# sag111/ContiniousEnvironment_Follower_Leader

Measured on AMD Instinct MI355X. Metric: env-steps/sec at 65,536 parallel envs; 1/2/4/8 MI355X scaling, higher is better.
Workload: dtype f64

## Files before the change

continiousenvironment_follower_leader_amd/_lib.py:

```python
import ctypes as C
import os
import subprocess

from . import abi

_PKG = os.path.dirname(os.path.abspath(__file__))
_ROOT = os.path.dirname(_PKG)
SO_PATH = os.path.join(_PKG, "libftl_hip.so")
SOURCES = [os.path.join(_PKG, "csrc", "ftl_abi.hip"), os.path.join(_PKG, "csrc", "ftl_device.hpp"),
           os.path.join(_PKG, "csrc", "ftl_frames_group.hpp"), os.path.join(_PKG, "csrc", "ftl_aux.hpp"), os.path.join(_PKG, "csrc", "ftl_gazebo.hpp"), os.path.join(_ROOT, "include", "ftl_gazebo.h"), os.path.join(_PKG, "csrc", "ftl_scenario.cpp"),
           os.path.join(_PKG, "csrc", "ftl_scenario_dev.hpp"),
           os.path.join(_PKG, "csrc", "ftl_scenario_core.hpp"),
           os.path.join(_PKG, "csrc", "ftl_crmath.hpp"),
           os.path.join(_PKG, "csrc", "ftl_render.hpp"),
           os.path.join(_PKG, "csrc", "ftl_snapshot.hpp"),
           os.path.join(_PKG, "csrc", "ftl_restart.hpp"),
           os.path.join(_PKG, "csrc", "ftl_queue.hpp"),
           os.path.join(_PKG, "csrc", "ftl_sampler.hpp"),
           os.path.join(_ROOT, "include", "ftl.h")]
UNITS = [os.path.join(_PKG, "csrc", "ftl_abi.hip"), os.path.join(_PKG, "csrc", "ftl_scenario.cpp")]
HIPCC = os.environ.get("HIPCC", "/opt/rocm/bin/hipcc")
HIPCC_FLAGS = ["--offload-arch=gfx950", "-O3", "-ffp-contract=off", "-fPIC", "-shared", "-std=c++17"]

_LIB = None


def build(force=False, verbose=False):
    stale = (not os.path.exists(SO_PATH)) or any(os.path.getmtime(s) > os.path.getmtime(SO_PATH) for s in SOURCES)
    if force or stale:
        cmd = [HIPCC] + HIPCC_FLAGS + ["-pthread", "-o", SO_PATH] + UNITS
        if verbose:
            print(" ".join(cmd))
        subprocess.check_call(cmd, cwd=os.path.join(_PKG, "csrc"))
    return SO_PATH


class FtlError(RuntimeError):
    pass


def load():
    global _LIB
# ... 106 lines not shown
```

continiousenvironment_follower_leader_amd/csrc/ftl_abi.hip:

```cpp
#include <hip/hip_runtime.h>

#include <cstdio>
#include <cstring>
#include <new>
#include <string>
#include <vector>

#include <cstdlib>
#include <cmath>

#include "ftl_device.hpp"
#include "ftl_frames_group.hpp"
#include "ftl_aux.hpp"

namespace {

thread_local std::string g_err;

int fail(int code, const std::string& msg) { g_err = msg; return code; }

struct Field { const char* name; size_t offset, per_env; int dtype; size_t stride; };

#define FTL_FIELDS(X) \
    X(rb_pos, 1, 4, true) X(rb_dbl, 2, 8, true) X(rb_int, 0, 4, true) X(env_int, 0, 4, true) X(env_dbl, 2, 8, true) \
    X(traj, 1, 4, false) X(hist, 2, 8, false) X(corr, 2, 8, false) X(snap_rects, 0, 4, true) X(snap_win, 0, 4, true) \
    X(traj_bb, 1, 4, false) X(ep_stats, 2, 8, false) X(hist1, 1, 4, false) X(fol_cs, 2, 8, true) X(corr32, 1, 4, false)
#define X(n, dtype, esz, rec) F_##n,
enum { FTL_FIELDS(X) FTL_N_FIELDS };
#undef X
struct FieldSpec { const char* name; int dtype; size_t esz; bool rec; size_t ptr; };
#define X(n, dtype, esz, rec) {#n, dtype, esz, rec, offsetof(FtlDevParams, n)},
constexpr FieldSpec kFields[FTL_N_FIELDS] = {FTL_FIELDS(X)};
#undef X
constexpr int kRecOrder[] = {F_env_int, F_fol_cs, F_rb_pos, F_rb_dbl, F_snap_win, F_snap_rects, F_env_dbl, F_rb_int};

struct Switches {
    int split, no_regroup, g8, one_pass, defer;
    int regroup_every, corr_lds_cap, lds_pad, lds_pad_rays;
    bool print_lds;
};

Switches read_switches() {
    auto tri = [](const char* name, int other) { const char* v = getenv(name); return !v ? -1 : v[0] == '1' ? 1 : v[0] == '0' ? 0 : other; };
    auto num = [](const char* name, int hi) { const char* v = getenv(name); const int p = v ? atoi(v) : 0; return p < 0 ? 0 : (p > hi ? hi : p); };
    return Switches{tri("FTL_SPLIT", 0), tri("FTL_NO_REGROUP", 0), tri("FTL_DEBUG_G8", 0), tri("FTL_RAYS_ONE_PASS", 1), tri("FTL_DEFER", 1),
                    num("FTL_REGROUP_EVERY", INT32_MAX), num("FTL_DEBUG_CORR_LDS_CAP", INT32_MAX), num("FTL_DEBUG_LDS_PAD", 48 * 1024),
                    num("FTL_DEBUG_LDS_PAD_RAYS", 48 * 1024), getenv("FTL_DEBUG_PRINT_LDS") != nullptr};
}

struct Schedule {
    int G, epw, rg_slots;
    int32_t fr_rec_off, fr_rec_stride, fr_pend_off, fr_env_off, fr_defer, fr_lds;
    bool regroup, fits;
};

struct FrameInst { int G; bool reg, xr; };
struct RaysInst { int hm; bool expl, split, capped, one_pass; };
typedef void (*FtlKernel)(const FtlDevParams*, const FtlCall);

}

template <typename T> struct FtlAttached { T v; bool attached; int32_t calls; };
struct FtlRestartScratch { int32_t* scen_idx; int32_t* list; uint8_t* ended; uint8_t* restarted; };

struct ftl_handle {
    FtlDevParams P;
    FtlDevParams* dP;
    bool dirty;
    int device;
    size_t state_bytes;
    Field fields[FTL_N_FIELDS];
    void* mt_mem;
    bool timing;
    std::vector<hipEvent_t> tev;
    size_t tev_used;
    bool bound, have_scen;
    Switches sw;
    Schedule sched;
    int co_envs, cus;
    bool one_pass;
    FtlKernel k_frames[2], k_rays[2]; RaysInst rays[2];
    bool has_aux, has_trk1;
    void* rg_mem;
    int* rg_tot;
    unsigned rg_parity, rg_launches, rg_every;
    hipStream_t side; hipEvent_t ev_fork, ev_join; bool split;
    int win_base, win_count, win_stride;
    float* last_lasers;
    FtlAttached<ftl_episode_queue> queue;
    FtlAttached<ftl_scenario_sampler> sampler;
// ... 51 lines not shown
        REQ(l.history > 0 && l.history <= FTL_HMAX, "laser %d: max_prev_obs must be in 1..%d", k, FTL_HMAX);
        REQ(l.react_obstacles >= 0 && l.react_obstacles <= 3, "laser %d: bad react_to_obstacles", k);
        REQ(l.length > 0, "laser %d: bad laser_length", k);
    }
#undef REQ
    return FTL_OK;
}

int frames_max(const ftl_config& c) { return c.rand_fps_hi > 0 ? c.rand_fps_hi - 1 : c.frames_per_step; }

Schedule plan_schedule(const ftl_config& cfg, int R, int n_envs, int co_envs, int cus, const Switches& sw) {
    Schedule s;
    s.G = (R > 4 || (sw.g8 >= 0 ? sw.g8 == 1 : co_envs <= cus * 4 * 8)) ? 8 : 4;
    s.epw = FTL_WAVE / s.G;
    const int f_max = frames_max(cfg);
    s.fr_defer = (cfg.rand_fps_hi == 0 && f_max >= 2 && f_max <= 16 && cfg.traj_cap <= 65535 && sw.defer != 0) ? 1 : 0;
    size_t o = align_up((size_t)s.epw * cfg.n_static * 16 + (size_t)s.epw * 4 + 32, 16);
    s.fr_rec_stride = (int)align_up((size_t)f_max, 16);
    s.fr_rec_off = (int)o; o += (size_t)s.fr_rec_stride * s.epw;
    s.fr_pend_off = (int)o; o += (size_t)s.epw * (s.fr_defer ? f_max - 1 : 1) * 16;
    s.fr_env_off = (int)o; o += (size_t)s.epw * 4 + 16 + (size_t)s.epw * 16;
    s.fr_lds = (int)o;
    s.fits = o <= 64 * 1024;
    s.rg_slots = cus * 4 * FTL_FRAMESG_WPE;
    s.regroup = (sw.no_regroup >= 0 ? sw.no_regroup == 0 : ((co_envs + s.epw - 1) / s.epw > s.rg_slots || cfg.rand_fps_hi > 0))
                && (n_envs + FTL_RG_BLOCK - 1) / FTL_RG_BLOCK <= 512;
    return s;
}

FrameInst frame_inst(const ftl_config& c, int G, bool xr) { return FrameInst{G, c.n_speed_regime >= 0 || c.n_acc_regime >= 0 || c.rand_fps_hi > 0, xr}; }

bool call_xr(const FtlCall& c) { return (c.flags & (FTL_STEP_NEXT_RESET | FTL_CALL_DEFER_RESET | FTL_CALL_FINISH)) != 0 || c.ended || c.restarted; }

RaysInst rays_inst(int hmax, bool expl, bool capped, bool two_streams, bool one_pass) {
    const int wide = hmax <= 5 ? 5 : FTL_HMAX;
    if (two_streams) return (!expl && hmax > 5 && hmax <= 10) ? RaysInst{10, false, true, capped, false} : RaysInst{wide, true, true, capped, false};
    if (expl) return RaysInst{wide, true, false, capped, false};
    return RaysInst{hmax <= 5 ? 5 : hmax <= 8 ? 8 : hmax <= 10 ? 10 : FTL_HMAX, false, false, capped, one_pass};
}

template <bool XR> FtlKernel frame_kernel_x(int G, bool reg) {
    if (G == 4) return reg ? ftl_frames_group_kernel<4, true, XR> : ftl_frames_group_kernel<4, false, XR>;
    return reg ? ftl_frames_group_kernel<8, true, XR> : ftl_frames_group_kernel<8, false, XR>;
}
FtlKernel frame_kernel(const FrameInst& f) { return f.xr ? frame_kernel_x<true>(f.G, f.reg) : frame_kernel_x<false>(f.G, f.reg); }

template <int HM, bool EXPL, bool SPLIT, bool ONE> FtlKernel rays_kernel_c(bool capped) {
    return capped ? ftl_rays_kernel<HM, EXPL, SPLIT, true, ONE> : ftl_rays_kernel<HM, EXPL, SPLIT, false, ONE>;
}
template <int HM> FtlKernel rays_kernel_1(const RaysInst& r) { return r.one_pass ? rays_kernel_c<HM, false, false, true>(r.capped) : rays_kernel_c<HM, false, false, false>(r.capped); }
FtlKernel rays_kernel(const RaysInst& r) {
    if (r.split) return r.hm == 10 ? rays_kernel_c<10, false, true, false>(r.capped) : r.hm == 5 ? rays_kernel_c<5, true, true, false>(r.capped) : rays_kernel_c<FTL_HMAX, true, true, false>(r.capped);
    if (r.expl) return r.hm == 5 ? rays_kernel_c<5, true, false, false>(r.capped) : rays_kernel_c<FTL_HMAX, true, false, false>(r.capped);
    return r.hm == 5 ? rays_kernel_1<5>(r) : r.hm == 8 ? rays_kernel_1<8>(r) : r.hm == 10 ? rays_kernel_1<10>(r) : rays_kernel_1<FTL_HMAX>(r);
}

int apply_plan(ftl_handle* h, int co_envs) {
    FtlDevParams& P = h->P;
    const ftl_config& c = P.cfg;
    const Schedule s = plan_schedule(c, P.R, P.n_envs, co_envs, h->cus, h->sw);
    if (!s.fits) return fail(FTL_E_INVALID, "the frame kernel needs more than 64 KiB of LDS per wavefront (static rects x frames per step)");
    h->sched = s; h->co_envs = co_envs; h->dirty = true;
    P.fr_rec_off = s.fr_rec_off; P.fr_rec_stride = s.fr_rec_stride; P.fr_pend_off = s.fr_pend_off; P.fr_env_off = s.fr_env_off;
    P.fr_defer = s.fr_defer; P.fr_lds = s.fr_lds;
    bool expl = false, compas = false;
    for (int k = 0; k < c.n_lasers; k++) { compas = compas || c.lasers[k].compas != 0; expl = expl || c.lasers[k].explicit_angles != 0 || c.lasers[k].pad_sectors != 0; }
    for (int i = 0; i < 2; i++) {
        h->k_frames[i] = frame_kernel(frame_inst(c, s.G, i == 1));
        h->rays[i] = rays_inst(P.hmax, expl || compas, P.corr_lds_cap < c.corr_cap, i == 1, h->one_pass);
        h->k_rays[i] = c.n_lasers > 0 ? rays_kernel(h->rays[i]) : nullptr;
    }
    h->has_aux = c.n_aux > 0 || compas; h->has_trk1 = c.has_tracker == 1;
    return FTL_OK;
}

void report_plan(const ftl_handle* h) {
    if (!h->sw.print_lds) return;
    const FtlDevParams& P = h->P;
    fprintf(stderr, "ftl: frame kernel LDS %d B per wavefront, %d lanes per env, %d frames at most, searches %s\n", P.fr_lds, h->sched.G, frames_max(P.cfg), P.fr_defer ? "deferred" : "in frame");
    fprintf(stderr, "ftl: ray kernel LDS %d B per env\n", P.lds_rays);
    char r[2][40] = {"no rays", "no rays"};
    for (int i = 0; i < 2; i++)
        if (h->k_rays[i]) snprintf(r[i], sizeof r[i], "rays<%d,%d,%d,%d,%d>", h->rays[i].hm, h->rays[i].expl, h->rays[i].split, h->rays[i].capped, h->rays[i].one_pass);
    fprintf(stderr, "ftl: kernels frames<%d,%d>, %s on one stream, %s on two; regroup %s every %u, two streams %s\n", h->sched.G, frame_inst(P.cfg, h->sched.G, false).reg,
            r[0], r[1], h->sched.regroup ? "on" : "off", h->rg_every, h->split ? "on" : "off");
}

}

extern "C" {

const char* ftl_last_error(void) { return g_err.c_str(); }

size_t ftl_sizeof_config(void) { return sizeof(ftl_config); }
size_t ftl_sizeof_scenarios(void) { return sizeof(ftl_scenarios); }
size_t ftl_sizeof_outputs(void) { return sizeof(ftl_outputs); }
size_t ftl_sizeof_scen_params(void) { return sizeof(ftl_scen_params); }
size_t ftl_sizeof_final_outputs(void) { return sizeof(ftl_final_outputs); }

int ftl_create(const ftl_config* cfg, int32_t n_envs, int32_t device, ftl_handle** out) {
    if (!cfg || !out) return fail(FTL_E_INVALID, "null argument");
    if (n_envs <= 0) return fail(FTL_E_INVALID, "n_envs must be positive");
    if (device < 0) return fail(FTL_E_INVALID, "device < 0: this library has no CPU path");
    std::string why;
    if (int rc = validate(*cfg, why)) return fail(rc, why);
    ftl_handle* h = new (std::nothrow) ftl_handle();
    if (!h) return fail(FTL_E_DEVICE, "out of host memory");
    h->P.cfg = *cfg;
    for (int k = 0; k < FTL_MAX_LASERS; k++) h->P.cfg.lasers[k].after_tracker = cfg->lasers[k].after_tracker ? 1 : 0;
    h->device = device; h->dirty = true;
    h->sw = read_switches();
    h->split = n_envs >= 8192 && (h->sw.split >= 0 ? h->sw.split == 1 : cfg->rand_fps_hi > 0) && cfg->has_tracker != 1;
    h->rg_every = h->sw.regroup_every > 0 ? (unsigned)h->sw.regroup_every : 4u;
    h->cus = 256;
    (void)hipDeviceGetAttribute(&h->cus, hipDeviceAttributeMultiprocessorCount, device);
    FtlDevParams& P = h->P;
    P.n_envs = n_envs;
    P.R = 2 + cfg->n_bears;
// ... 23 lines not shown
        }
        P.miss_const = miss_ok ? 1 : 0;
        int rb[2] = {0, 0};
        for (int k = 0; k < cfg->n_lasers; k++) {
            const ftl_laser_cfg& l = cfg->lasers[k];
            FtlRaySensor& rs = P.ray_sens[k];
            const int which = l.after_tracker ? 1 : 0, ro = l.react_obstacles;
            rs.count = l.count; rs.rbase = rb[which];
            rs.reach2 = ((float)l.length + 2.0f) * ((float)l.length + 2.0f);
            rs.inv_step = (float)l.count * 0.15915494309189535f; rs.inv_count = 1.0f / (float)l.count;
            rs.off_u = (float)(l.angle_offset * deg2rad) * rs.inv_step;
            rs.slack = 0.022f + 0.01f * (float)l.count * 0.15915494f;
            rs.flags = ((ro == 1 || ro == 2) ? 1u : 0u) | ((ro == 1 || ro == 3) ? 2u : 0u) | (l.react_corridor ? 4u : 0u) | (l.react_green ? 8u : 0u)
                     | (l.explicit_angles ? 16u : 0u) | (which ? 32u : 0u) | (l.compas ? 64u : 0u);
            if (!l.compas) rb[which] += l.count;
        }
        P.inv_nrect_dyn = (65536u + (unsigned)(P.R - 1) - 1u) / (unsigned)(P.R - 1);
        int g = 0;
        for (int which = 0; which < 2; which++) {
            P.pass_base[which] = g; P.pass_lmax[which] = 0.0f;
            for (int k = 0; k < cfg->n_lasers; k++) {
                const ftl_laser_cfg& l = cfg->lasers[k];
                if ((l.after_tracker ? 1 : 0) != which || l.compas) continue;
                P.pass_lmax[which] = fmaxf(P.pass_lmax[which], (float)l.length);
                for (int i = 0; i < l.count && g < FTL_MAX_RAYS; i++, g++) {
                    const double a = l.explicit_angles ? l.ray_angles[i & 7] : l.angle_offset + i * (360.0 / (double)l.count);
                    P.ray_dir[g].c = cos(a * deg2rad); P.ray_dir[g].s = sin(a * deg2rad); P.ray_dir[g].len = l.length;
                }
            }
            P.pass_rays[which] = g - P.pass_base[which];
        }
        P.pass_single = P.pass_rays[0] > 0 && P.pass_rays[1] > 0 ? -1 : (P.pass_rays[1] > 0 ? 1 : 0);
        h->one_pass = P.pass_single >= 0 && h->sw.one_pass != 0;
    }
    if (rays > 1023) { delete h; return fail(FTL_E_INVALID, "more than 1023 rays per env (the candidate list of the ray kernel packs a ray index into 10 bits)"); }
    if (hmax * (P.R - 1) > FTL_WAVE) { delete h; return fail(FTL_E_INVALID, "max_prev_obs x (1 + bears) exceeds one wavefront of snapshot rects"); }
    {
        int w = 0, hcommon = 0;
        for (int k = 0; k < cfg->n_lasers; k++) {
            P.pol_off[k] = -1;
            if (!cfg->lasers[k].in_policy_obs) continue;
            P.pol_off[k] = w; w += width_of(cfg->lasers[k]);
            if (hcommon == 0) hcommon = cfg->lasers[k].history;
            else if (cfg->lasers[k].history != hcommon) hcommon = -1;
        }
        P.pol_width = w; P.pol_h = hcommon;
    }
    const size_t n = (size_t)n_envs;
    size_t per_env[FTL_N_FIELDS];
    per_env[F_rb_pos] = (size_t)P.R * 2; per_env[F_rb_dbl] = (size_t)P.R * FTL_RD_COUNT; per_env[F_rb_int] = (size_t)P.R * FTL_RI_COUNT;
    per_env[F_env_int] = FTL_EI_COUNT; per_env[F_env_dbl] = FTL_ED_COUNT; per_env[F_fol_cs] = 2;
    per_env[F_snap_rects] = (size_t)hmax * (P.R - 1) * 4; per_env[F_snap_win] = (size_t)hmax * 4;
    per_env[F_traj] = (size_t)cfg->traj_cap * 2; per_env[F_traj_bb] = (size_t)(cfg->traj_cap / FTL_TRAJ_BLOCK) * 4;
    per_env[F_hist] = (size_t)cfg->corr_cap * 2; per_env[F_corr] = (size_t)cfg->corr_cap * 4; per_env[F_corr32] = (size_t)cfg->corr_cap * 4;
    per_env[F_hist1] = (size_t)(cfg->has_tracker == 1 ? cfg->hist1_cap : 0) * 2; per_env[F_ep_stats] = FTL_N_METRICS;
    size_t ro = 0;
    for (int i : kRecOrder) {
        ro = align_up(ro, 16);
        h->fields[i] = Field{kFields[i].name, ro, per_env[i], kFields[i].dtype, 0};
        ro += per_env[i] * kFields[i].esz;
    }
    const size_t rec_stride = align_up(ro, 128);
    P.rec_stride = (int32_t)rec_stride;
    for (int i : kRecOrder) h->fields[i].stride = rec_stride;
    size_t cur = rec_stride * n;
    for (int i = 0; i < FTL_N_FIELDS; i++) {
        if (kFields[i].rec) continue;
        cur = align_up(cur, 256);
        h->fields[i] = Field{kFields[i].name, cur, per_env[i], kFields[i].dtype, per_env[i] * kFields[i].esz};
        cur += per_env[i] * kFields[i].esz * n;
    }
    h->state_bytes = align_up(cur, 256);
    {
        const size_t rects = (size_t)cfg->n_static + hmax + (size_t)hmax * (P.R - 2 > 0 ? P.R - 2 : 0) + 1;
        P.corr_lds_cap = cfg->corr_cap < 128 ? cfg->corr_cap : 128;
        if (const int v = h->sw.corr_lds_cap; v >= 2 && v <= cfg->corr_cap && (v & (v - 1)) == 0) P.corr_lds_cap = v;
        const int hm_lds = rays_inst(hmax, true, false, false, false).hm;
        P.lds_rays = (int)((size_t)P.corr_lds_cap * 16 + rects * 20 + (size_t)2 * P.corr_lds_cap * 4 + (size_t)2 * hmax * 20 + 64
                           + (size_t)rays * 16 + (size_t)rays * hm_lds * 4 + (size_t)rays * 4
                           + rects * 8 + 32
                           + (size_t)FTL_PAIR_CAP * 2 + 16);
    }
    P.lds_rays += h->sw.lds_pad_rays;
    if (cfg->traj_cap > 65535 || frames_max(*cfg) > 4095) { delete h; return fail(FTL_E_INVALID, "traj_cap above 65535 or more than 4095 frames per step"); }
    if (apply_plan(h, n_envs)) { delete h; return FTL_E_INVALID; }
    report_plan(h);
    if (P.lds_rays > 64 * 1024) { delete h; return fail(FTL_E_INVALID, "config needs more than 64 KiB of LDS per env"); }
    if (ftl_aux_lds_bytes(*cfg) > 64 * 1024) { delete h; return fail(FTL_E_INVALID, "the compas / lidar / radar sensors of this config need more than 64 KiB of LDS per env"); }
    *out = h;
    return FTL_OK;
}

void ftl_destroy(ftl_handle* h) {
    if (!h) return;
    if (h->dP || h->rg_mem || h->side || h->mt_mem || h->rs.scen_idx) (void)hipSetDevice(h->device);
    if (h->rs.scen_idx) (void)hipFree(h->rs.scen_idx);
    if (h->dP) (void)hipFree(h->dP);
    if (h->mt_mem) (void)hipFree(h->mt_mem);
    for (hipEvent_t ev : h->tev) (void)hipEventDestroy(ev);
    if (h->rg_mem) (void)hipFree(h->rg_mem);
    if (h->side) { (void)hipStreamSynchronize(h->side); (void)hipStreamDestroy(h->side); }
    if (h->ev_fork) (void)hipEventDestroy(h->ev_fork);
    if (h->ev_join) (void)hipEventDestroy(h->ev_join);
    delete h;
}

int32_t ftl_lasers_len(const ftl_handle* h) { return h ? h->P.lasers_len : 0; }

int ftl_get_config(const ftl_handle* h, ftl_config* out) {
    if (!h || !out) return fail(FTL_E_INVALID, "null argument");
// ... 315 lines not shown
```

continiousenvironment_follower_leader_amd/csrc/ftl_device.hpp:

```cpp
#pragma once
#include <hip/hip_runtime.h>
#include <stddef.h>
#include <stdint.h>

#include "../../include/ftl.h"

#define FTL_WAVE 64
#define FTL_HMAX 12
#define FTL_MAX_RAYS 1024
#ifndef FTL_WIDE_ARC
#define FTL_WIDE_ARC 3
#endif
#define FTL_PAIR_CAP (64 * FTL_WIDE_ARC)
#ifndef FTL_RAYS_WPE
#define FTL_RAYS_WPE 6
#endif

struct FtlRaySensor {
    int32_t count, rbase;
    float reach2;
    float inv_step, inv_count;
    float off_u;
    float slack;
    uint32_t flags;
};
struct alignas(16) FtlRayDir { double c, s, len, _pad; };
struct FtlDevParams {
    ftl_config cfg;
    int32_t n_envs, R, lasers_len, total_rays, hmax, lds_rays;
    int32_t pass_rays[2], pass_base[2];
    float pass_lmax[2];
    int32_t pass_single;
    int32_t _pad_pass;
    int32_t fr_rec_off, fr_rec_stride, fr_pend_off, fr_env_off, fr_defer, fr_lds;
    int32_t corr_lds_cap;
    int32_t pol_off[FTL_MAX_LASERS], pol_width, pol_h;
    float* rb_pos; double* rb_dbl; int32_t* rb_int; int32_t* env_int; double* env_dbl;
    int32_t rec_stride, _pad_rec;
    float* traj; double* hist; double* corr; int32_t* snap_rects; int32_t* snap_win;
    float* traj_bb;
    double* ep_stats;
    float* corr32;
    float* hist1;
    double* fol_cs;
    FtlRayDir ray_dir[FTL_MAX_RAYS];
    FtlRaySensor ray_sens[FTL_MAX_LASERS];
    uint32_t inv_nrect_dyn;
    int32_t miss_const;
    int32_t* perm; uint8_t* keys; uint16_t* rank; int32_t* bh;
    ftl_scenarios scen;
};
static_assert(sizeof(FtlRayDir) == 32 && offsetof(FtlDevParams, ray_dir) % 32 == 0, "ray_dir: 16-byte loads of its records must be aligned, and a record must not straddle a cache line (the device copy is 256-byte aligned)");
struct FtlCall {
    const double* action; const int32_t* scen_idx; const uint8_t* mask;
    ftl_outputs out;
    uint32_t flags; int32_t mode;
    int32_t action_kind;
    int32_t win_base, win_count, win_stride;
    int32_t part, parts, epw;
    uint8_t* ended; uint8_t* restarted;
};
#define FTL_CALL_DEFER_RESET (1u << 30)
#define FTL_CALL_FINISH (1u << 29)
#define FTL_CALL_SCEN_IDX (1u << 28)

template <typename T>
// ... 240 lines not shown
    double t = (double)num / denom;
    double x = t * rbx + (double)cx, y = t * rby + (double)cy;
    double qx = x - (double)cx, qy = y - (double)cy;
    d2 = qx * qx + qy * qy;
    return true;
}

}

__device__ __forceinline__ float arc_atan2(float y, float x) {
    const float ax = fabsf(x), ay = fabsf(y);
    const bool steep = ay > ax;
    const float hi = steep ? ay : ax, lo = steep ? ax : ay;
    const float a = hi > 0.0f ? lo * __builtin_amdgcn_rcpf(hi) : 0.0f;
    const float t = a * a;
    float r = a * __builtin_fmaf(t, __builtin_fmaf(t, __builtin_fmaf(t, __builtin_fmaf(t, 0.0208351f, -0.0851330f), 0.1801410f), -0.3302995f), 0.9998660f);
    r = steep ? 1.5707963267948966f - r : r;
    r = x < 0.0f ? 3.141592653589793f - r : r;
    return y < 0.0f ? -r : r;
}

#ifdef FTL_PROFILE_RAYS
__device__ unsigned long long g_rcyc[16];
__shared__ unsigned long long s_rcyc[16];
#define FTL_RTIC(slot) do { unsigned long long _t = __builtin_readcyclecounter(); if (threadIdx.x == 0) s_rcyc[slot] += _t - _rprev; _rprev = _t; } while (0)
#define FTL_RTIC_INIT unsigned long long _rprev = __builtin_readcyclecounter()
#else
#define FTL_RTIC(slot) do { } while (0)
#define FTL_RTIC_INIT do { } while (0)
#endif

#define FTL_FOR_LASERS(k) _Pragma("unroll") for (int k = 0; k < FTL_MAX_LASERS; k++) if (k < c.n_lasers && !(EXPL && c.lasers[k].compas))

template <int HM, bool EXPL = false, bool SPLIT = false, bool CAPPED = false, bool ONE_PASS = false>
__global__ void __launch_bounds__(FTL_WAVE, FTL_RAYS_WPE) ftl_rays_kernel(const FtlDevParams* __restrict__ Pp, const FtlCall C) {
    extern __shared__ __align__(16) unsigned char lds[];
    using namespace ftl;
    const FtlDevParams& P = *Pp;
    const ftl_config& c = P.cfg;
    int env = blockIdx.x;
    if (SPLIT) {
        const int gslot = ((int)(blockIdx.x / C.epw) * C.parts + C.part) * C.epw + (int)(blockIdx.x % C.epw);
        if (gslot >= P.n_envs) return;
        env = P.perm ? P.perm[gslot] : gslot;
    }
    if (env >= P.n_envs) return;
    if (C.mode == 1 && C.mask && !C.mask[env]) return;
    const int lane = threadIdx.x;
#ifdef FTL_PROFILE_RAYS
    if (lane < 16) s_rcyc[lane] = 0;
    __syncthreads();
#endif
    FTL_RTIC_INIT;
    const int hmax = P.hmax;
    const int nrect_dyn = P.R - 1;
    const int cmask = P.corr_lds_cap - 1;
    const int cap_rs = c.n_static + hmax, cap_rd = hmax * (P.R - 2 > 0 ? P.R - 2 : 0) + 1;
    const int cap_cr = 2 * P.corr_lds_cap, cap_gr = 2 * hmax;
    float4* s_corr = reinterpret_cast<float4*>(lds);
    int4* s_rect = reinterpret_cast<int4*>(s_corr + P.corr_lds_cap);
    float4* s_green = reinterpret_cast<float4*>(s_rect + cap_rs + cap_rd);
    unsigned* s_rmask = reinterpret_cast<unsigned*>(s_green + cap_gr);
    unsigned* s_cref = s_rmask + cap_rs + cap_rd;
    unsigned* s_gmask = s_cref + cap_cr;
    int* s_cnt = reinterpret_cast<int*>(s_gmask + cap_gr);
    int* s_ecnt = s_cnt + SEG_CLASSES;
    unsigned short* s_edge = reinterpret_cast<unsigned short*>(s_cnt + 8);
    const int n_u32 = (cap_rs + cap_rd) + cap_cr + cap_gr + 8 + 2 * (cap_rs + cap_rd);
// ... 168 lines not shown
                    const int at = ent >> 2;
                    const int4 q = s_rect[at]; sm = s_rmask[at];
                    const float l = (float)q.x, t = (float)q.y, r = (float)(q.x + q.z), b = (float)(q.y + q.w);
                    const int e = ent & 3;
                    sg = e == 0 ? make_float4(l, b, r, b) : e == 1 ? make_float4(r, t, r, b) : e == 2 ? make_float4(r, t, l, t) : make_float4(l, b, l, t);
                } else if (mq == SEG_CORRIDOR) {
                    if (staged) {
                        const unsigned ref = s_cref[m];
                        const int p = ref & 0x7fff; sm = ref >> 16;
                        const float4 u = s_corr[p], v = s_corr[(p + 1) & cmask];
                        sg = (ref >> 15) & 1u ? make_float4(u.z, u.w, v.z, v.w) : make_float4(u.x, u.y, v.x, v.y);
                    } else {
                        const int p = umin + (m >> 1);
                        sm = 0;
#pragma unroll
                        for (int a = 0; a < HM; a++) if (a < nsnap && win_lo[a] <= p && p + 1 < win_hi[a]) sm |= 1u << a;
                        const float4 u = corr_f32(p), v = corr_f32(p + 1);
                        sg = (m & 1) ? make_float4(u.z, u.w, v.z, v.w) : make_float4(u.x, u.y, v.x, v.y);
                    }
                } else { sg = s_green[m]; sm = s_gmask[m]; }
            };
            auto test = [&](int ray, const float4& sgx, unsigned smx) {
                const double2 e = s_ray[ray];
                double d2;
                if (hit_segment(cx, cy, e.x, e.y, (float)e.x, (float)e.y, sgx, d2)) {
                    d2 = sqrt(d2);
                    const unsigned bits = __float_as_uint((float)d2);
#pragma unroll
                    for (int j = 0; j < HM; j++) if ((smx >> j) & 1u) atomicMin(&s_best[j * P.total_rays + ray], bits);
                }
            };
            const float fdir_rad = (float)(fdir * kDeg2Rad);
            int np_u = 0;
            for (int w0 = 0; w0 < n_items; w0 += FTL_WAVE) {
                const int w = w0 + lane;
                int m = -1, mq = 0;
                {
                    int j = 0, start = 0, end = 0;
#pragma unroll
                    for (int q = 0; q < SEG_CLASSES; q++) {
                        end += cq[q];
                        const bool past = w >= end;
                        j += past ? 1 : 0; start = past ? end : start;
                    }
                    if (w < n_items) { m = w - start; mq = j; }
                }
                FTL_RTIC(3);
                float4 sg = make_float4(0.f, 0.f, 0.f, 0.f); unsigned sm = 0;
                float a0 = 0.0f, wd = 0.0f, dmin2 = 3.0e38f;
                if (m >= 0) {
                    fetch(mq, m, sg, sm);
                    if (sm == 0u) m = -1;
                }
                if (m >= 0) {
                    const float ax = sg.x - cx, ay = sg.y - cy, bx = sg.z - cx, by = sg.w - cy;
                    const float angA = arc_atan2(ay, ax), angB = arc_atan2(by, bx);
                    float diff = angB - angA; if (diff < 0.0f) diff += 6.283185307179586f;
                    a0 = angA; wd = diff;
                    if (diff > 3.141592653589793f) { a0 = angB; wd = 6.283185307179586f - diff; }
                    a0 -= fdir_rad;
                    const float ex_ = bx - ax, ey_ = by - ay;
                    const float l2 = __builtin_fmaf(ex_, ex_, ey_ * ey_);
                    const float tt = l2 > 0.0f ? fminf(fmaxf(-__builtin_fmaf(ax, ex_, ay * ey_) * __builtin_amdgcn_rcpf(l2), 0.0f), 1.0f) : 0.0f;
                    const float nx = __builtin_fmaf(tt, ex_, ax), ny = __builtin_fmaf(tt, ey_, ay);
                    dmin2 = __builtin_fmaf(nx, nx, ny * ny);
                }
                FTL_RTIC(4);
                auto flush = [&](int np) {
                    __syncthreads();
                    for (int p0 = 0; p0 < np; p0 += FTL_WAVE) {
                        const int p = p0 + lane;
                        const unsigned rec = p < np ? s_pair[p] : 0u;
                        const int L = (int)(rec >> 10);
                        const float4 sgp = make_float4(__shfl(sg.x, L), __shfl(sg.y, L), __shfl(sg.z, L), __shfl(sg.w, L));
                        const unsigned smp = (unsigned)__shfl((int)sm, L);
                        if (p < np) test((int)(rec & 1023u), sgp, smp);
                    }
                    __syncthreads();
                };
#pragma nounroll
                for (int k = 0; k < c.n_lasers; k++) {
                    const FtlRaySensor rs = P.ray_sens[k];
                    if ((int)((rs.flags >> 5) & 1u) != which || (rs.flags & 64u)) continue;
                    const int N = rs.count, rbase = rs.rbase;
                    int i0 = 0, cnt = 0;
                    if (m >= 0 && ((rs.flags >> mq) & 1u) && !(dmin2 > rs.reach2)) {
                        const float fN = (float)N;
                        const float wu = wd * rs.inv_step;
                        if ((rs.flags & 16u) || dmin2 < 4.0f || wu > 0.5f * fN - 0.05f) { i0 = 0; cnt = N; }
                        else {
                            float st = __builtin_fmaf(a0, rs.inv_step, -rs.off_u);
                            st = __builtin_fmaf(-floorf(st * rs.inv_count), fN, st);
                            i0 = (int)ceilf(st - rs.slack);
                            cnt = (int)floorf(st + wu + rs.slack) - i0 + 1;
                            cnt = cnt > N ? N : cnt;
                        }
                    }
#if defined(FTL_RAYS_STOP) && FTL_RAYS_STOP == 5
                    cnt = cnt == 0x7fffffff ? 1 : 0;
#endif
#ifdef FTL_PROFILE_RAYS
                    if (threadIdx.x == 0) { s_rcyc[8] += 1; }
                    { int mc = cnt; for (int o = 32; o >= 1; o >>= 1) mc = max(mc, __shfl_xor(mc, o)); int ni = __popcll(__ballot(m >= 0)); int sc = cnt; for (int o = 32; o >= 1; o >>= 1) sc += __shfl_xor(sc, o); if (threadIdx.x == 0) { s_rcyc[9] += mc; s_rcyc[10] += sc; s_rcyc[11] += ni; s_rcyc[12] += (mc <= 2); s_rcyc[13] += (mc > 2 && mc <= 4); s_rcyc[14] += (mc > 4 && mc <= 8); s_rcyc[15] += (mc > 8); } }
#endif
                    unsigned long long wide = __ballot(cnt > FTL_WIDE_ARC);
                    while (wide) {
                        const int L = __ffsll((long long)wide) - 1; wide &= wide - 1;
                        const int i0L = __builtin_amdgcn_readlane(i0, L), cntL = __builtin_amdgcn_readlane(cnt, L);
                        if (cntL > FTL_WAVE) {
                            const float4 sgL = make_float4(__int_as_float(__builtin_amdgcn_readlane(__float_as_int(sg.x), L)), __int_as_float(__builtin_amdgcn_readlane(__float_as_int(sg.y), L)),
                                                           __int_as_float(__builtin_amdgcn_readlane(__float_as_int(sg.z), L)), __int_as_float(__builtin_amdgcn_readlane(__float_as_int(sg.w), L)));
                            const unsigned smL = (unsigned)__builtin_amdgcn_readlane((int)sm, L);
                            for (int t = lane; t < cntL; t += FTL_WAVE) {
                                int i = i0L + t; i = i < 0 ? i + N : (i >= N ? i - N : i);
                                test(rbase + i, sgL, smL);
                            }
                            continue;
                        }
                        if (np_u + cntL > FTL_PAIR_CAP) { flush(np_u); np_u = 0; }
                        if (lane < cntL) {
                            int i = i0L + lane; i = i < 0 ? i + N : (i >= N ? i - N : i);
                            s_pair[np_u + lane] = (unsigned short)((L << 10) | (rbase + i));
                        }
                        np_u += cntL;
                    }
                    const int own = cnt > FTL_WIDE_ARC ? 0 : cnt;
                    int pre = 0, tot = 0;
#pragma unroll
                    for (int b = 0; b < 4; b++) if ((FTL_WIDE_ARC >> b) != 0) {
                        const unsigned long long bm = __ballot((own >> b) & 1);
                        pre += (int)__builtin_amdgcn_mbcnt_hi((unsigned)(bm >> 32), __builtin_amdgcn_mbcnt_lo((unsigned)bm, 0u)) << b;
                        tot += __popcll(bm) << b;
                    }
                    if (np_u + tot > FTL_PAIR_CAP) { flush(np_u); np_u = 0; }
                    for (int t = 0; t < own; t++) {
                        int i = i0 + t; i = i < 0 ? i + N : (i >= N ? i - N : i);
                        s_pair[np_u + pre + t] = (unsigned short)((lane << 10) | (rbase + i));
                    }
                    np_u += tot;
                }
                if (np_u > 0) { flush(np_u); np_u = 0; }
            }
        }
        FTL_RTIC(5);
#if defined(FTL_RAYS_STOP) && FTL_RAYS_STOP == 4
        continue;
#endif
        __syncthreads();
        {
            float* pol = C.out.policy_obs ? C.out.policy_obs + (size_t)env * P.pol_h * P.pol_width : nullptr;
            bool any_pad = false;
            FTL_FOR_LASERS(k) if (EXPL && c.lasers[k].after_tracker == which && c.lasers[k].pad_sectors) {
                any_pad = true;
                const int tot = c.lasers[k].history * 4 * c.lasers[k].count;
                for (int i = lane; i < tot; i += FTL_WAVE) out_base[c.lasers[k].out_offset + i] = 0.0f;
                if (pol && P.pol_off[k] >= 0) for (int i = lane; i < tot; i += FTL_WAVE) {
                    int row = i / (4 * c.lasers[k].count), col = i - row * 4 * c.lasers[k].count;
                    pol[row * P.pol_width + P.pol_off[k] + col] = 0.0f;
                }
            }
            if (any_pad) __syncthreads();
            if constexpr (!EXPL) {
                for (int g = lane; g < n_rays; g += FTL_WAVE) {
                    int i = g, H = 0, N = 0, ooff = 0, poff = -1; float flen = 1.0f; bool found = false;
                    FTL_FOR_LASERS(k) if (c.lasers[k].after_tracker == which) {
                        const int Nk = c.lasers[k].count;
                        if (!found && i < Nk) {
                            found = true; N = Nk; H = c.lasers[k].history; ooff = c.lasers[k].out_offset; poff = P.pol_off[k];
                            flen = (float)c.lasers[k].length;
                        }
                        if (!found) i -= Nk;
                    }
                    const float miss = s_miss[g];
#pragma unroll
// ... 43 lines not shown
```

Baseline: 272.5 million.

## Build ray candidate pairs from per-lane 64-bit ray masks in one-pass kernel

When a pass has at most 64 rays, each lane now ORs the ray arcs of all sensors into one 64-bit mask. It then computes its slot with a DPP wavefront prefix sum and writes the candidate pairs in windows of configurable size. This replaces the per-sensor ballot and readlane loop, the wide-arc special path and the repeated flush checks. The cost is serial per-lane bit extraction, which can leave lanes unevenly loaded.

After: 282.0 million (median of 6 runs). 1.03x the previous value.

```diff
diff --git a/continiousenvironment_follower_leader_amd/_lib.py b/continiousenvironment_follower_leader_amd/_lib.py
--- a/continiousenvironment_follower_leader_amd/_lib.py
+++ b/continiousenvironment_follower_leader_amd/_lib.py
@@ -8,6 +8,7 @@
 _ROOT = os.path.dirname(_PKG)
 SO_PATH = os.path.join(_PKG, "libftl_hip.so")
 SOURCES = [os.path.join(_PKG, "csrc", "ftl_abi.hip"), os.path.join(_PKG, "csrc", "ftl_device.hpp"),
+           os.path.join(_PKG, "csrc", "ftl_raymask.hpp"),
            os.path.join(_PKG, "csrc", "ftl_frames_group.hpp"), os.path.join(_PKG, "csrc", "ftl_aux.hpp"), os.path.join(_PKG, "csrc", "ftl_gazebo.hpp"), os.path.join(_ROOT, "include", "ftl_gazebo.h"), os.path.join(_PKG, "csrc", "ftl_scenario.cpp"),
            os.path.join(_PKG, "csrc", "ftl_scenario_dev.hpp"),
            os.path.join(_PKG, "csrc", "ftl_scenario_core.hpp"),
diff --git a/continiousenvironment_follower_leader_amd/csrc/ftl_abi.hip b/continiousenvironment_follower_leader_amd/csrc/ftl_abi.hip
--- a/continiousenvironment_follower_leader_amd/csrc/ftl_abi.hip
+++ b/continiousenvironment_follower_leader_amd/csrc/ftl_abi.hip
@@ -37,6 +37,7 @@
 struct Switches {
     int split, no_regroup, g8, one_pass, defer;
     int regroup_every, corr_lds_cap, lds_pad, lds_pad_rays;
+    int pair_window;
     bool print_lds;
 };
 
@@ -45,7 +46,7 @@
     auto num = [](const char* name, int hi) { const char* v = getenv(name); const int p = v ? atoi(v) : 0; return p < 0 ? 0 : (p > hi ? hi : p); };
     return Switches{tri("FTL_SPLIT", 0), tri("FTL_NO_REGROUP", 0), tri("FTL_DEBUG_G8", 0), tri("FTL_RAYS_ONE_PASS", 1), tri("FTL_DEFER", 1),
                     num("FTL_REGROUP_EVERY", INT32_MAX), num("FTL_DEBUG_CORR_LDS_CAP", INT32_MAX), num("FTL_DEBUG_LDS_PAD", 48 * 1024),
-                    num("FTL_DEBUG_LDS_PAD_RAYS", 48 * 1024), getenv("FTL_DEBUG_PRINT_LDS") != nullptr};
+                    num("FTL_DEBUG_LDS_PAD_RAYS", 48 * 1024), num("FTL_DEBUG_PAIR_WINDOW", FTL_PAIR_CAP), getenv("FTL_DEBUG_PRINT_LDS") != nullptr};
 }
 
 struct Schedule {
@@ -55,7 +56,7 @@
 };
 
 struct FrameInst { int G; bool reg, xr; };
-struct RaysInst { int hm; bool expl, split, capped, one_pass; };
+struct RaysInst { int hm; bool expl, split, capped, one_pass, mask; };
 typedef void (*FtlKernel)(const FtlDevParams*, const FtlCall);
 
 }
@@ -173,11 +174,11 @@
 
 bool call_xr(const FtlCall& c) { return (c.flags & (FTL_STEP_NEXT_RESET | FTL_CALL_DEFER_RESET | FTL_CALL_FINISH)) != 0 || c.ended || c.restarted; }
 
-RaysInst rays_inst(int hmax, bool expl, bool capped, bool two_streams, bool one_pass) {
+RaysInst rays_inst(int hmax, bool expl, bool capped, bool two_streams, bool one_pass, int pass_rays) {
     const int wide = hmax <= 5 ? 5 : FTL_HMAX;
-    if (two_streams) return (!expl && hmax > 5 && hmax <= 10) ? RaysInst{10, false, true, capped, false} : RaysInst{wide, true, true, capped, false};
-    if (expl) return RaysInst{wide, true, false, capped, false};
-    return RaysInst{hmax <= 5 ? 5 : hmax <= 8 ? 8 : hmax <= 10 ? 10 : FTL_HMAX, false, false, capped, one_pass};
+    if (two_streams) return (!expl && hmax > 5 && hmax <= 10) ? RaysInst{10, false, true, capped, false, false} : RaysInst{wide, true, true, capped, false, false};
+    if (expl) return RaysInst{wide, true, false, capped, false, false};
+    return RaysInst{hmax <= 5 ? 5 : hmax <= 8 ? 8 : hmax <= 10 ? 10 : FTL_HMAX, false, false, capped, one_pass, one_pass && pass_rays <= 64};
 }
 
 template <bool XR> FtlKernel frame_kernel_x(int G, bool reg) {
@@ -186,10 +187,13 @@
 }
 FtlKernel frame_kernel(const FrameInst& f) { return f.xr ? frame_kernel_x<true>(f.G, f.reg) : frame_kernel_x<false>(f.G, f.reg); }
 
-template <int HM, bool EXPL, bool SPLIT, bool ONE> FtlKernel rays_kernel_c(bool capped) {
-    return capped ? ftl_rays_kernel<HM, EXPL, SPLIT, true, ONE> : ftl_rays_kernel<HM, EXPL, SPLIT, false, ONE>;
-}
-template <int HM> FtlKernel rays_kernel_1(const RaysInst& r) { return r.one_pass ? rays_kernel_c<HM, false, false, true>(r.capped) : rays_kernel_c<HM, false, false, false>(r.capped); }
+template <int HM, bool EXPL, bool SPLIT, bool ONE, bool MASK = false> FtlKernel rays_kernel_c(bool capped) {
+    return capped ? ftl_rays_kernel<HM, EXPL, SPLIT, true, ONE, MASK> : ftl_rays_kernel<HM, EXPL, SPLIT, false, ONE, MASK>;
+}
+template <int HM> FtlKernel rays_kernel_1(const RaysInst& r) {
+    if (r.mask) return rays_kernel_c<HM, false, false, true, true>(r.capped);
+    return r.one_pass ? rays_kernel_c<HM, false, false, true>(r.capped) : rays_kernel_c<HM, false, false, false>(r.capped);
+}
 FtlKernel rays_kernel(const RaysInst& r) {
     if (r.split) return r.hm == 10 ? rays_kernel_c<10, false, true, false>(r.capped) : r.hm == 5 ? rays_kernel_c<5, true, true, false>(r.capped) : rays_kernel_c<FTL_HMAX, true, true, false>(r.capped);
     if (r.expl) return r.hm == 5 ? rays_kernel_c<5, true, false, false>(r.capped) : rays_kernel_c<FTL_HMAX, true, false, false>(r.capped);
@@ -208,7 +212,7 @@
     for (int k = 0; k < c.n_lasers; k++) { compas = compas || c.lasers[k].compas != 0; expl = expl || c.lasers[k].explicit_angles != 0 || c.lasers[k].pad_sectors != 0; }
     for (int i = 0; i < 2; i++) {
         h->k_frames[i] = frame_kernel(frame_inst(c, s.G, i == 1));
-        h->rays[i] = rays_inst(P.hmax, expl || compas, P.corr_lds_cap < c.corr_cap, i == 1, h->one_pass);
+        h->rays[i] = rays_inst(P.hmax, expl || compas, P.corr_lds_cap < c.corr_cap, i == 1, h->one_pass, h->one_pass ? P.pass_rays[P.pass_single] : 0);
         h->k_rays[i] = c.n_lasers > 0 ? rays_kernel(h->rays[i]) : nullptr;
     }
     h->has_aux = c.n_aux > 0 || compas; h->has_trk1 = c.has_tracker == 1;
@@ -225,6 +229,7 @@
         if (h->k_rays[i]) snprintf(r[i], sizeof r[i], "rays<%d,%d,%d,%d,%d>", h->rays[i].hm, h->rays[i].expl, h->rays[i].split, h->rays[i].capped, h->rays[i].one_pass);
     fprintf(stderr, "ftl: kernels frames<%d,%d>, %s on one stream, %s on two; regroup %s every %u, two streams %s\n", h->sched.G, frame_inst(P.cfg, h->sched.G, false).reg,
             r[0], r[1], h->sched.regroup ? "on" : "off", h->rg_every, h->split ? "on" : "off");
+    if (h->k_rays[0]) fprintf(stderr, "     ray candidates: %s form on one stream, %s form on two, window %d\n", h->rays[0].mask ? "mask" : "list", h->rays[1].mask ? "mask" : "list", P.pair_window);
 }
 
 }
@@ -314,6 +319,8 @@
         }
         P.pass_single = P.pass_rays[0] > 0 && P.pass_rays[1] > 0 ? -1 : (P.pass_rays[1] > 0 ? 1 : 0);
         h->one_pass = P.pass_single >= 0 && h->sw.one_pass != 0;
+        P.pair_window = FTL_PAIR_CAP;
+        if (const int v = h->sw.pair_window; v >= 16 && v <= FTL_PAIR_CAP && v % 16 == 0) P.pair_window = v;
     }
     if (rays > 1023) { delete h; return fail(FTL_E_INVALID, "more than 1023 rays per env (the candidate list of the ray kernel packs a ray index into 10 bits)"); }
     if (hmax * (P.R - 1) > FTL_WAVE) { delete h; return fail(FTL_E_INVALID, "max_prev_obs x (1 + bears) exceeds one wavefront of snapshot rects"); }
@@ -357,7 +364,7 @@
         const size_t rects = (size_t)cfg->n_static + hmax + (size_t)hmax * (P.R - 2 > 0 ? P.R - 2 : 0) + 1;
         P.corr_lds_cap = cfg->corr_cap < 128 ? cfg->corr_cap : 128;
         if (const int v = h->sw.corr_lds_cap; v >= 2 && v <= cfg->corr_cap && (v & (v - 1)) == 0) P.corr_lds_cap = v;
-        const int hm_lds = rays_inst(hmax, true, false, false, false).hm;
+        const int hm_lds = rays_inst(hmax, true, false, false, false, 0).hm;
         P.lds_rays = (int)((size_t)P.corr_lds_cap * 16 + rects * 20 + (size_t)2 * P.corr_lds_cap * 4 + (size_t)2 * hmax * 20 + 64
                            + (size_t)rays * 16 + (size_t)rays * hm_lds * 4 + (size_t)rays * 4
                            + rects * 8 + 32
diff --git a/continiousenvironment_follower_leader_amd/csrc/ftl_device.hpp b/continiousenvironment_follower_leader_amd/csrc/ftl_device.hpp
--- a/continiousenvironment_follower_leader_amd/csrc/ftl_device.hpp
+++ b/continiousenvironment_follower_leader_amd/csrc/ftl_device.hpp
@@ -4,6 +4,7 @@
 #include <stdint.h>
 
 #include "../../include/ftl.h"
+#include "ftl_raymask.hpp"
 
 #define FTL_WAVE 64
 #define FTL_HMAX 12
@@ -31,7 +32,7 @@
     int32_t pass_rays[2], pass_base[2];
     float pass_lmax[2];
     int32_t pass_single;
-    int32_t _pad_pass;
+    int32_t pair_window;
     int32_t fr_rec_off, fr_rec_stride, fr_pend_off, fr_env_off, fr_defer, fr_lds;
     int32_t corr_lds_cap;
     int32_t pol_off[FTL_MAX_LASERS], pol_width, pol_h;
@@ -338,8 +339,9 @@
 
 #define FTL_FOR_LASERS(k) _Pragma("unroll") for (int k = 0; k < FTL_MAX_LASERS; k++) if (k < c.n_lasers && !(EXPL && c.lasers[k].compas))
 
-template <int HM, bool EXPL = false, bool SPLIT = false, bool CAPPED = false, bool ONE_PASS = false>
+template <int HM, bool EXPL = false, bool SPLIT = false, bool CAPPED = false, bool ONE_PASS = false, bool MASK = false>
 __global__ void __launch_bounds__(FTL_WAVE, FTL_RAYS_WPE) ftl_rays_kernel(const FtlDevParams* __restrict__ Pp, const FtlCall C) {
+    static_assert(!MASK || (ONE_PASS && !EXPL && !SPLIT), "the mask form of phase 3 exists for the one-pass, one-stream kernels of the common sensors");
     extern __shared__ __align__(16) unsigned char lds[];
     using namespace ftl;
     const FtlDevParams& P = *Pp;
@@ -574,6 +576,7 @@
             };
             const float fdir_rad = (float)(fdir * kDeg2Rad);
             int np_u = 0;
+            const int win = MASK ? min(max(P.pair_window, 16), FTL_PAIR_CAP) : FTL_PAIR_CAP;
             for (int w0 = 0; w0 < n_items; w0 += FTL_WAVE) {
                 const int w = w0 + lane;
                 int m = -1, mq = 0;
@@ -620,68 +623,116 @@
                     }
                     __syncthreads();
                 };
+                if constexpr (MASK) {
+                    unsigned long long mk = 0ull;
 #pragma nounroll
-                for (int k = 0; k < c.n_lasers; k++) {
-                    const FtlRaySensor rs = P.ray_sens[k];
-                    if ((int)((rs.flags >> 5) & 1u) != which || (rs.flags & 64u)) continue;
-                    const int N = rs.count, rbase = rs.rbase;
-                    int i0 = 0, cnt = 0;
-                    if (m >= 0 && ((rs.flags >> mq) & 1u) && !(dmin2 > rs.reach2)) {
-                        const float fN = (float)N;
-                        const float wu = wd * rs.inv_step;
-                        if ((rs.flags & 16u) || dmin2 < 4.0f || wu > 0.5f * fN - 0.05f) { i0 = 0; cnt = N; }
-                        else {
-                            float st = __builtin_fmaf(a0, rs.inv_step, -rs.off_u);
-                            st = __builtin_fmaf(-floorf(st * rs.inv_count), fN, st);
-                            i0 = (int)ceilf(st - rs.slack);
-                            cnt = (int)floorf(st + wu + rs.slack) - i0 + 1;
-                            cnt = cnt > N ? N : cnt;
+                    for (int k = 0; k < c.n_lasers; k++) {
+                        const FtlRaySensor rs = P.ray_sens[k];
+                        if ((int)((rs.flags >> 5) & 1u) != which || (rs.flags & 64u)) continue;
+                        const int N = rs.count;
+                        int i0 = 0, cnt = 0;
+                        if (m >= 0 && ((rs.flags >> mq) & 1u) && !(dmin2 > rs.reach2)) {
+                            const float fN = (float)N;
+                            const float wu = wd * rs.inv_step;
+                            if ((rs.flags & 16u) || dmin2 < 4.0f || wu > 0.5f * fN - 0.05f) { i0 = 0; cnt = N; }
+                            else {
+                                float st = __builtin_fmaf(a0, rs.inv_step, -rs.off_u);
+                                st = __builtin_fmaf(-floorf(st * rs.inv_count), fN, st);
+                                i0 = (int)ceilf(st - rs.slack);
+                                cnt = (int)floorf(st + wu + rs.slack) - i0 + 1;
+                                cnt = cnt > N ? N : cnt;
+                            }
                         }
+                        mk |= ftl_ray_mask(i0, cnt, N, rs.rbase);
                     }
 #if defined(FTL_RAYS_STOP) && FTL_RAYS_STOP == 5
-                    cnt = cnt == 0x7fffffff ? 1 : 0;
-#endif
+                    mk = mk == ~0ull - 1ull ? 1ull : 0ull;
+#endif
+                    const int cntm = __popcll(mk);
+                    int inc = cntm;
+                    inc += __builtin_amdgcn_update_dpp(0, inc, 0x111, 0xf, 0xf, false);
+                    inc += __builtin_amdgcn_update_dpp(0, inc, 0x112, 0xf, 0xf, false);
+                    inc += __builtin_amdgcn_update_dpp(0, inc, 0x114, 0xf, 0xf, false);
+                    inc += __builtin_amdgcn_update_dpp(0, inc, 0x118, 0xf, 0xf, false);
+                    inc += __builtin_amdgcn_update_dpp(0, inc, 0x142, 0xa, 0xf, false);
+                    inc += __builtin_amdgcn_update_dpp(0, inc, 0x143, 0xc, 0xf, false);
+                    const int tot = __builtin_amdgcn_readlane(inc, FTL_WAVE - 1);
+                    const int pos = inc - cntm;
 #ifdef FTL_PROFILE_RAYS
-                    if (threadIdx.x == 0) { s_rcyc[8] += 1; }
-                    { int mc = cnt; for (int o = 32; o >= 1; o >>= 1) mc = max(mc, __shfl_xor(mc, o)); int ni = __popcll(__ballot(m >= 0)); int sc = cnt; for (int o = 32; o >= 1; o >>= 1) sc += __shfl_xor(sc, o); if (threadIdx.x == 0) { s_rcyc[9] += mc; s_rcyc[10] += sc; s_rcyc[11] += ni; s_rcyc[12] += (mc <= 2); s_rcyc[13] += (mc > 2 && mc <= 4); s_rcyc[14] += (mc > 4 && mc <= 8); s_rcyc[15] += (mc > 8); } }
-#endif
-                    unsigned long long wide = __ballot(cnt > FTL_WIDE_ARC);
-                    while (wide) {
-                        const int L = __ffsll((long long)wide) - 1; wide &= wide - 1;
-                        const int i0L = __builtin_amdgcn_readlane(i0, L), cntL = __builtin_amdgcn_readlane(cnt, L);
-                        if (cntL > FTL_WAVE) {
-                            const float4 sgL = make_float4(__int_as_float(__builtin_amdgcn_readlane(__float_as_int(sg.x), L)), __int_as_float(__builtin_amdgcn_readlane(__float_as_int(sg.y), L)),
-                                                           __int_as_float(__builtin_amdgcn_readlane(__float_as_int(sg.z), L)), __int_as_float(__builtin_amdgcn_readlane(__float_as_int(sg.w), L)));
-                            const unsigned smL = (unsigned)__builtin_amdgcn_readlane((int)sm, L);
-                            for (int t = lane; t < cntL; t += FTL_WAVE) {
-                                int i = i0L + t; i = i < 0 ? i + N : (i >= N ? i - N : i);
-                                test(rbase + i, sgL, smL);
+                    { int mc = cntm; for (int o = 32; o >= 1; o >>= 1) mc = max(mc, __shfl_xor(mc, o)); const int ni = __popcll(__ballot(m >= 0)); if (threadIdx.x == 0) { s_rcyc[8] += 1ull + (w0 == FTL_WAVE ? 1ull << 40 : 0ull);  s_rcyc[9] += mc; s_rcyc[10] += tot; s_rcyc[11] += ni; s_rcyc[12] += (mc <= 2); s_rcyc[13] += (mc > 2 && mc <= 4); s_rcyc[14] += (mc > 4 && mc <= 8); s_rcyc[15] += (mc > 8); } }
+#endif
+                    unsigned lo = (unsigned)mk, hi = (unsigned)(mk >> 32);
+                    const unsigned tag = (unsigned)lane << 10;
+                    unsigned rel = (unsigned)pos;
+                    for (int wb = 0; wb < tot; wb += win, rel -= (unsigned)win) {
+                        while (lo != 0u && rel < (unsigned)win) { s_pair[rel++] = (unsigned short)(tag | (unsigned)(__ffs(lo) - 1)); lo &= lo - 1u; }
+                        while (hi != 0u && rel < (unsigned)win) { s_pair[rel++] = (unsigned short)(tag | (unsigned)(__ffs(hi) + 31)); hi &= hi - 1u; }
+                        flush(min(tot - wb, win));
+                    }
+                } else {
+#pragma nounroll
+                    for (int k = 0; k < c.n_lasers; k++) {
+                        const FtlRaySensor rs = P.ray_sens[k];
+                        if ((int)((rs.flags >> 5) & 1u) != which || (rs.flags & 64u)) continue;
+                        const int N = rs.count, rbase = rs.rbase;
+                        int i0 = 0, cnt = 0;
+                        if (m >= 0 && ((rs.flags >> mq) & 1u) && !(dmin2 > rs.reach2)) {
+                            const float fN = (float)N;
+                            const float wu = wd * rs.inv_step;
+                            if ((rs.flags & 16u) || dmin2 < 4.0f || wu > 0.5f * fN - 0.05f) { i0 = 0; cnt = N; }
+                            else {
+                                float st = __builtin_fmaf(a0, rs.inv_step, -rs.off_u);
+                                st = __builtin_fmaf(-floorf(st * rs.inv_count), fN, st);
+                                i0 = (int)ceilf(st - rs.slack);
+                                cnt = (int)floorf(st + wu + rs.slack) - i0 + 1;
+                                cnt = cnt > N ? N : cnt;
                             }
-                            continue;
                         }
-                        if (np_u + cntL > FTL_PAIR_CAP) { flush(np_u); np_u = 0; }
-                        if (lane < cntL) {
-                            int i = i0L + lane; i = i < 0 ? i + N : (i >= N ? i - N : i);
-                            s_pair[np_u + lane] = (unsigned short)((L << 10) | (rbase + i));
+#if defined(FTL_RAYS_STOP) && FTL_RAYS_STOP == 5
+                        cnt = cnt == 0x7fffffff ? 1 : 0;
+#endif
+#ifdef FTL_PROFILE_RAYS
+                        if (threadIdx.x == 0) { s_rcyc[8] += 1; }
+                        { int mc = cnt; for (int o = 32; o >= 1; o >>= 1) mc = max(mc, __shfl_xor(mc, o)); int ni = __popcll(__ballot(m >= 0)); int sc = cnt; for (int o = 32; o >= 1; o >>= 1) sc += __shfl_xor(sc, o); if (threadIdx.x == 0) { s_rcyc[9] += mc; s_rcyc[10] += sc; s_rcyc[11] += ni; s_rcyc[12] += (mc <= 2); s_rcyc[13] += (mc > 2 && mc <= 4); s_rcyc[14] += (mc > 4 && mc <= 8); s_rcyc[15] += (mc > 8); } }
+#endif
+                        unsigned long long wide = __ballot(cnt > FTL_WIDE_ARC);
+                        while (wide) {
+                            const int L = __ffsll((long long)wide) - 1; wide &= wide - 1;
+                            const int i0L = __builtin_amdgcn_readlane(i0, L), cntL = __builtin_amdgcn_readlane(cnt, L);
+                            if (cntL > FTL_WAVE) {
+                                const float4 sgL = make_float4(__int_as_float(__builtin_amdgcn_readlane(__float_as_int(sg.x), L)), __int_as_float(__builtin_amdgcn_readlane(__float_as_int(sg.y), L)),
+                                                               __int_as_float(__builtin_amdgcn_readlane(__float_as_int(sg.z), L)), __int_as_float(__builtin_amdgcn_readlane(__float_as_int(sg.w), L)));
+                                const unsigned smL = (unsigned)__builtin_amdgcn_readlane((int)sm, L);
+                                for (int t = lane; t < cntL; t += FTL_WAVE) {
+                                    int i = i0L + t; i = i < 0 ? i + N : (i >= N ? i - N : i);
+                                    test(rbase + i, sgL, smL);
+                                }
+                                continue;
+                            }
+                            if (np_u + cntL > FTL_PAIR_CAP) { flush(np_u); np_u = 0; }
+                            if (lane < cntL) {
+                                int i = i0L + lane; i = i < 0 ? i + N : (i >= N ? i - N : i);
+                                s_pair[np_u + lane] = (unsigned short)((L << 10) | (rbase + i));
+                            }
+                            np_u += cntL;
                         }
-                        np_u += cntL;
+                        const int own = cnt > FTL_WIDE_ARC ? 0 : cnt;
+                        int pre = 0, tot = 0;
+#pragma unroll
+                        for (int b = 0; b < 4; b++) if ((FTL_WIDE_ARC >> b) != 0) {
+                            const unsigned long long bm = __ballot((own >> b) & 1);
+                            pre += (int)__builtin_amdgcn_mbcnt_hi((unsigned)(bm >> 32), __builtin_amdgcn_mbcnt_lo((unsigned)bm, 0u)) << b;
+                            tot += __popcll(bm) << b;
+                        }
+                        if (np_u + tot > FTL_PAIR_CAP) { flush(np_u); np_u = 0; }
+                        for (int t = 0; t < own; t++) {
+                            int i = i0 + t; i = i < 0 ? i + N : (i >= N ? i - N : i);
+                            s_pair[np_u + pre + t] = (unsigned short)((lane << 10) | (rbase + i));
+                        }
+                        np_u += tot;
                     }
-                    const int own = cnt > FTL_WIDE_ARC ? 0 : cnt;
-                    int pre = 0, tot = 0;
-#pragma unroll
-                    for (int b = 0; b < 4; b++) if ((FTL_WIDE_ARC >> b) != 0) {
-                        const unsigned long long bm = __ballot((own >> b) & 1);
-                        pre += (int)__builtin_amdgcn_mbcnt_hi((unsigned)(bm >> 32), __builtin_amdgcn_mbcnt_lo((unsigned)bm, 0u)) << b;
-                        tot += __popcll(bm) << b;
-                    }
-                    if (np_u + tot > FTL_PAIR_CAP) { flush(np_u); np_u = 0; }
-                    for (int t = 0; t < own; t++) {
-                        int i = i0 + t; i = i < 0 ? i + N : (i >= N ? i - N : i);
-                        s_pair[np_u + pre + t] = (unsigned short)((lane << 10) | (rbase + i));
-                    }
-                    np_u += tot;
-                }
-                if (np_u > 0) { flush(np_u); np_u = 0; }
+                    if (np_u > 0) { flush(np_u); np_u = 0; }
+                }
             }
         }
         FTL_RTIC(5);
diff --git a/continiousenvironment_follower_leader_amd/csrc/ftl_raymask.hpp b/continiousenvironment_follower_leader_amd/csrc/ftl_raymask.hpp
--- /dev/null
+++ b/continiousenvironment_follower_leader_amd/csrc/ftl_raymask.hpp
@@ -0,0 +1,22 @@
+#pragma once
+#include <stdint.h>
+
+#if defined(__HIPCC__) || defined(__CUDACC__)
+#define FTL_RAYMASK_FN __host__ __device__ __forceinline__
+#else
+#define FTL_RAYMASK_FN inline
+#endif
+
+FTL_RAYMASK_FN uint64_t ftl_ray_mask(int i0, int cnt, int N, int rbase) {
+    const int s = i0 < 0 ? i0 + N : (i0 >= N ? i0 - N : i0);
+    if (N <= 32) {
+        const uint32_t ones = cnt >= 32 ? 0xffffffffu : (1u << cnt) - 1u;
+        const uint32_t field = N >= 32 ? 0xffffffffu : (1u << N) - 1u;
+        const uint32_t f = ((ones << s) | ((ones >> 1) >> (N - 1 - s))) & field;
+        return (uint64_t)f << rbase;
+    }
+    const uint64_t ones = cnt >= 64 ? ~0ull : (1ull << cnt) - 1ull;
+    const uint64_t field = N >= 64 ? ~0ull : (1ull << N) - 1ull;
+    const uint64_t f = ((ones << s) | ((ones >> 1) >> (N - 1 - s))) & field;
+    return f << rbase;
+}
```
